# wienkers/marEx

Hardware: AMD Instinct MI355X
Metric: Mcells*timesteps/s, shifting_baseline + hobday_extreme p95 (validation+anomaly+thresholds+mask) (higher is better)
Workload: dtype f32

## Files before the change

### include/marex_hip.h

```cpp
#ifndef MAREX_HIP_H
#define MAREX_HIP_H

#include <stddef.h>
#include <stdint.h>

#ifdef __cplusplus
extern "C" {
#endif

#define MAREX_ABI_VERSION 2
#define MAREX_NDOY 366

typedef struct marex_ctx marex_ctx;

typedef struct marex_thr_stats {
    uint32_t min_key;
    uint32_t max_key;
    uint32_t n_too_low;
    uint32_t n_too_high;
    uint32_t n_unresolved;
    uint32_t reserved[3];
} marex_thr_stats;

enum {
// ... 11 lines not shown
    MAREX_K_TAILS = 11,
    MAREX_K_COUNT = 12
};

int marex_abi_version(void);

typedef struct marex_workspace_cfg {
    int64_t T;
    int64_t T_out;
    int64_t C;
    int max_bucket;
    int list_rows;
} marex_workspace_cfg;
enum {
    MAREX_WS_ANOMALY = 0,
    MAREX_WS_EXTREME = 1,
    MAREX_WS_THRESHOLDS = 2,
    MAREX_WS_LISTS = 3,
    MAREX_WS_AUX = 4,
    MAREX_WS_BINS = 5,
    MAREX_WS_PER_CELL = 6,
    MAREX_WS_TOTAL = 7,
    MAREX_WS_COUNT = 8
};
int marex_workspace_bytes(const marex_workspace_cfg* cfg, size_t* bytes);
int marex_create(int device, marex_ctx** out);
int marex_destroy(marex_ctx* ctx);
const char* marex_last_error(marex_ctx* ctx);
int marex_set_stream(marex_ctx* ctx, void* hip_stream);
int marex_sync(marex_ctx* ctx);

int marex_set_option(marex_ctx* ctx, const char* name, int value);
int marex_clear_option(marex_ctx* ctx, const char* name);
int marex_debug_counters(marex_ctx* ctx, uint64_t* out8, int reset);

int marex_timing_enable(marex_ctx* ctx, int on);
int marex_timing_reset(marex_ctx* ctx);
int marex_timing_get(marex_ctx* ctx, int kernel_id, double* total_ms, int64_t* launches);

int marex_synth_sst_f32(marex_ctx* ctx, const float* mean, const float* amp, const uint8_t* hemi,
                        const uint8_t* land, const float* seas , const float* trend ,
                        uint64_t seed, int64_t cell_base, int64_t T, int64_t C, float* x );

int marex_shifting_baseline_f32(marex_ctx* ctx, const float* x, int64_t T, int64_t C,
                                const int32_t* year_plan, int n_cal_years, int W, int S,
                                int write_clim, const float* edges, int nb, int64_t T_out, float* out,
                                uint16_t* bins, uint8_t* mask, int32_t* invalid_count);

int marex_hobday_thresholds_f32(marex_ctx* ctx, const uint16_t* bins, int64_t T_out, int64_t C, int ny,
                                int nx, const int32_t* doy_start, int max_bucket, const float* first_anom,
                                const float* centres, int nb, double q, int wd, int ws,
                                float lower_bound, float upper_bound, int row0, int row1,
                                float* thr_doy_major, marex_thr_stats* stats);

int marex_mask_ge_doy_f32(marex_ctx* ctx, const float* anom, const float* thr_doy_major,
                          const int32_t* doy_start, const int32_t* doy_rows, int64_t T_out, int64_t C,
                          int64_t c0, int64_t c1, uint8_t* extreme, unsigned long long* n_true);

int marex_mask_ge_doy_bins_f32(marex_ctx* ctx, const float* anom, const uint16_t* bins, const float* edges, int nb,
                               const float* thr_doy_major, const int32_t* doy_start, const int32_t* doy_rows, int64_t T_out,
                               int64_t C, int64_t c0, int64_t c1, uint8_t* extreme, unsigned long long* n_true);

int marex_tail_lists(int max_bucket, int list_rows);
int marex_tail_extract_f32(marex_ctx* ctx, const float* anom, int64_t T_out, int64_t C, const int32_t* doy_start,
                           const int32_t* doy_rows, int max_bucket, const float* edges, int nb, int list_rows, void* lists,
                           uint32_t* aux);

// ... 163 lines not shown
```

### marex_amd/_lib.py

```python

from __future__ import annotations

import ctypes as C
import os
from typing import Optional

from .exceptions import DependencyError, ProcessingError

_HERE = os.path.dirname(os.path.abspath(__file__))
LIB_PATH = os.environ.get("MAREX_LIB_PATH") or os.path.join(_HERE, "csrc", "libmarex_hip.so")

_p = C.c_void_p
_i32 = C.c_int
_i64 = C.c_int64
_u64 = C.c_uint64
_f32 = C.c_float
_f64 = C.c_double

PROTOTYPES = {
    "marex_abi_version": (_i32, []),
    "marex_workspace_bytes": (_i32, [_p, _p]),
    "marex_create": (_i32, [_i32, C.POINTER(_p)]),
    "marex_destroy": (_i32, [_p]),
    "marex_last_error": (C.c_char_p, [_p]),
# ... 163 lines not shown
            raise ProcessingError(f"{what} failed (code {rc})", details=msg.decode() if msg else None)

    def set_stream(self, stream_ptr: int) -> None:
        self.check(self.lib.marex_set_stream(self.handle, _p(stream_ptr)), "marex_set_stream")

    def sync(self) -> None:
        self.check(self.lib.marex_sync(self.handle), "marex_sync")

    def set_option(self, name: str, value: Optional[int]) -> None:
        if value is None:
            self.check(self.lib.marex_clear_option(self.handle, name.encode()), "marex_clear_option")
            self.py_opts.pop(name, None)
        else:
            self.check(self.lib.marex_set_option(self.handle, name.encode(), int(value)), "marex_set_option")
            self.py_opts[name] = int(value)

    def options(self, **opts):
        import contextlib

        @contextlib.contextmanager
        def _cm():
            before = {k: self.py_opts.get(k) for k in opts}
            for k, v in opts.items():
                self.set_option(k, v)
            try:
                yield self
            finally:
                for k, old in before.items():
                    self.set_option(k, old)

        return _cm()

    def debug_counters(self, reset: bool = True):
        buf = (C.c_uint64 * 8)()
        self.check(self.lib.marex_debug_counters(self.handle, buf, int(reset)), "marex_debug_counters")
        return [int(v) for v in buf]

    def timing_enable(self, on: bool = True) -> None:
        self.check(self.lib.marex_timing_enable(self.handle, int(on)), "marex_timing_enable")

    def timing_reset(self) -> None:
        self.check(self.lib.marex_timing_reset(self.handle), "marex_timing_reset")

    def timing_get(self, kernel: str):
        ms, n = _f64(0.0), _i64(0)
        self.check(
            self.lib.marex_timing_get(self.handle, KERNEL_IDS[kernel], C.byref(ms), C.byref(n)), "marex_timing_get"
        )
        return ms.value, n.value
```

### marex_amd/csrc/marex_common.hip.h

```cpp
#pragma once
#include <hip/hip_runtime.h>

#include <cmath>
#include <type_traits>
#include <cstdarg>
#include <cstdio>
#include <cstring>
#include <map>
#include <string>
#include <vector>

#include "marex_hip.h"

#define NDOY MAREX_NDOY

struct TimedLaunch {
    int kid;
    hipEvent_t a, b;
};

struct marex_ctx {
    int device = 0;
    hipStream_t stream = nullptr;
    std::string err;
    bool timing = false;
    std::vector<TimedLaunch> pending;
    double total_ms[MAREX_K_COUNT] = {0};
    int64_t launches[MAREX_K_COUNT] = {0};
    int* shift_info = nullptr;
    int* shift_plan = nullptr;
    size_t shift_plan_years = 0;
    int* shift_lplan = nullptr;
    size_t shift_lplan_years = 0;
    unsigned char* thr_scratch = nullptr;
    size_t thr_scratch_bytes = 0;
    unsigned char* detrend_scratch = nullptr;
    size_t detrend_scratch_bytes = 0;
    unsigned char* morph_scratch = nullptr;
    size_t morph_scratch_bytes = 0;
    int n_cu = 0;
    std::map<std::string, int> opts;
    long long* row_off = nullptr;
    size_t row_off_bytes = 0;
    long long* row_off_mask = nullptr;
    size_t row_off_mask_bytes = 0;
    unsigned long long* dbg_counters = nullptr;
};

#define MAREX_DBG_COUNTERS 8

static inline int ctx_opt(marex_ctx* ctx, const char* name, int dflt) {
    auto it = ctx->opts.find(name);
    return it == ctx->opts.end() ? dflt : it->second;
}

#ifdef MAREX_ABLATION
#define MAREX_ABLATE_OPT(ctx, name) ctx_opt(ctx, name, 0)
#else
#define MAREX_ABLATE_OPT(ctx, name) 0
#endif

static inline unsigned long long* ctx_debug_counters(marex_ctx* ctx) {
    if (!ctx->dbg_counters) {
        if (hipMalloc((void**)&ctx->dbg_counters, MAREX_DBG_COUNTERS * sizeof(unsigned long long)) != hipSuccess) return nullptr;
        (void)hipMemsetAsync(ctx->dbg_counters, 0, MAREX_DBG_COUNTERS * sizeof(unsigned long long), ctx->stream);
    }
    return ctx->dbg_counters;
}

static inline int device_cus(marex_ctx* ctx) {
    if (ctx->n_cu <= 0) {
        int n = 0;
        if (hipDeviceGetAttribute(&n, hipDeviceAttributeMultiprocessorCount, ctx->device) != hipSuccess || n <= 0) n = 256;
        ctx->n_cu = n;
    }
    return ctx->n_cu;
}

static inline int fail(marex_ctx* ctx, int code, const char* fmt, ...) {
    char buf[512];
    va_list ap;
    va_start(ap, fmt);
// ... 131 lines not shown
```

### marex_amd/csrc/marex_tails.hip

```cpp
#include "marex_common.hip.h"
#include "marex_tails.hip.h"

typedef __amdgpu_buffer_rsrc_t tl_rsrc_t;
__device__ __forceinline__ tl_rsrc_t tl_make_rsrc(const void* base) {
    return __builtin_amdgcn_make_buffer_rsrc(const_cast<void*>(base), 0, -1, 0x00020000);
}
__device__ __forceinline__ uint4 tl_load_chunk(tl_rsrc_t r, unsigned voff, unsigned soff) {
    typedef unsigned u4 __attribute__((ext_vector_type(4)));
    const u4 v = __builtin_amdgcn_raw_buffer_load_b128(r, (int)voff, (int)soff, 0);
    return make_uint4(v.x, v.y, v.z, v.w);
}
__device__ __forceinline__ unsigned pk_sub_sat_u16(unsigned a, unsigned b) {
    unsigned r;
    asm("v_pk_sub_u16 %0, %1, %2 clamp" : "=v"(r) : "v"(a), "v"(b));
    return r;
}
__device__ __forceinline__ unsigned pk_add_u16(unsigned a, unsigned b) {
    unsigned r;
    asm("v_pk_add_u16 %0, %1, %2" : "=v"(r) : "v"(a), "v"(b));
    return r;
}
__device__ __forceinline__ unsigned pk_sub_u16(unsigned a, unsigned b) {
    unsigned r;
    asm("v_pk_sub_u16 %0, %1, %2" : "=v"(r) : "v"(a), "v"(b));
// ... 303 lines not shown
        cell = (long)j * nx + gi;
    } else {
        cell_valid = icol < nx && !spare;
        cell = icol < nx ? icol : nx - 1;
    }
    if (!cell_valid) cell = 0;
    const bool is_out = !spare && tr >= P && tr < TR - P && tc >= P && tc < TC - P && j < row1 && icol < nx && (ny > 0 ? j >= row0 : true);
    const int d_begin = (int)blockIdx.y * Dd;
    const int ndays = (NDOY - d_begin) < Dd ? (NDOY - d_begin) : Dd;
    const int pd = wd / 2;
    bool land = true;
    if (is_out) land = !(anom[cell] == anom[cell]);
    if (!__syncthreads_or(is_out && !land)) {
        if (is_out)
            for (int dd = 0; dd < ndays; ++dd) thr[(size_t)(d_begin + dd) * C + cell] = nan_f();
        return;
    }
    if (is_out && land)
        for (int dd = 0; dd < ndays; ++dd) thr[(size_t)(d_begin + dd) * C + cell] = nan_f();

    unsigned* mycol = &lev[ci * TT_LS];
    uint2* mycol2 = reinterpret_cast<uint2*>(mycol);
    typedef __attribute__((address_space(3))) unsigned lds_u32;
    const unsigned col_lds = (unsigned)(size_t)(lds_u32*)mycol;
    const int base_max = nb - TT_BW > 0 ? nb - TT_BW : 0;
    auto clamp_base = [&](int b) { return b < 0 ? 0 : (b > base_max ? base_max : b); };
    int B0 = 0;
    int BW = nb < TT_BW ? nb : TT_BW;
    constexpr int NLP = (TT_BW + 2 + 1) / 2;
    const unsigned voff = (unsigned)cell * 16u;
    const unsigned chunk_row = (unsigned)C * 16u;
    const size_t day_stride = (size_t)NPER * nch * (size_t)C;

    auto load_bucket = [&](int d0) {
        TailBucket<NPERT> b;
        b.d = d0;
        const tl_rsrc_t r = tl_make_rsrc(lists + (size_t)d0 * day_stride);
#pragma unroll
        for (int p = 0; p < NPF; ++p)
            b.c0[p] = (p < NPER) ? tl_load_chunk(r, voff, (unsigned)(nch * p) * chunk_row) : make_uint4(0, 0, 0, 0);
        b.aux = aux[(size_t)d0 * C + cell];
        return b;
    };
    auto bump = [&](int k, int sgn) {
        const int odd = k & 1;
        unsigned addr;
        asm("v_lshl_add_u32 %0, %1, 1, %2" : "=v"(addr) : "v"(k - odd), "v"(col_lds));
        int v;
        const int mul = sgn > 0 ? 65535 : -65535, one = sgn > 0 ? 1 : -1;
        asm("v_mad_i32_i24 %0, %1, %2, %3" : "=v"(v) : "v"(odd), "v"(mul), "v"(one));
        __hip_atomic_fetch_add((lds_u32*)(size_t)addr, (unsigned)v, __ATOMIC_RELAXED, __HIP_MEMORY_SCOPE_WORKGROUP);
    };
    int mytot = 0;
    constexpr bool ctx_asm_bump = true;
    auto bump_chunk = [&](const uint4& ch, int n, int sgn, int nfix) {
#pragma unroll
        for (int u = 0; u < 8; ++u) {
            const bool on = n > u;
            if (u >= nfix && __builtin_amdgcn_ballot_w64(on) == 0) break;
            if (on) {
                int lvl = tl_bin1(ch, u) - B0;
                lvl = lvl > BW + 1 ? BW + 1 : lvl;
                bump(lvl, sgn);
            }
        }
    };
    auto apply_bucket = [&](const TailBucket<NPERT>& b, int sgn) {
        const int cnt = cell_valid ? (int)(b.aux & 0x3FFu) : 0;
        const unsigned lim = ((unsigned)(B0 + 1) << TAIL_POS_BITS) - 1u;
        const unsigned lim_rep = lim | (lim << 16);
        const tl_rsrc_t r = tl_make_rsrc(lists + (size_t)b.d * day_stride);
        int n_in = 0;
        auto one_list = [&](const uint4& ch, int p) {
            const int n = cnt > 0 ? tl_count_above(ch, lim_rep) : 0;
            n_in += n;
            if (ctx_asm_bump) { if (sgn > 0) tl_bump_chunk<1>(ch, n, B0, BW + 1, col_lds); else tl_bump_chunk<-1>(ch, n, B0, BW + 1, col_lds); }
            else bump_chunk(ch, n, sgn, NPERT >= 3 ? 2 : 1);
            bool full = n == 8;
#pragma unroll
            for (int jj = 1; jj < 4; ++jj) {
                if (jj >= nch || __builtin_amdgcn_ballot_w64(full) == 0) break;
                const uint4 cj = tl_load_chunk(r, voff, (unsigned)(nch * p + jj) * chunk_row);
                const int nj = full ? tl_count_above(cj, lim_rep) : 0;
                n_in += nj;
                if (ctx_asm_bump) { if (sgn > 0) tl_bump_chunk<1>(cj, nj, B0, BW + 1, col_lds); else tl_bump_chunk<-1>(cj, nj, B0, BW + 1, col_lds); }
                else bump_chunk(cj, nj, sgn, 0);
                full = nj == 8;
            }
        };
#pragma unroll
        for (int p = 0; p < NPF; ++p)
            if (p < NPER) one_list(b.c0[p], p);
#pragma nounroll
        for (int p = NPF; p < NPER; p += 2) {
            const uint4 e0 = tl_load_chunk(r, voff, (unsigned)(nch * p) * chunk_row);
            const uint4 e1 = p + 1 < NPER ? tl_load_chunk(r, voff, (unsigned)(nch * (p + 1)) * chunk_row) : make_uint4(0, 0, 0, 0);
            one_list(e0, p);
            if (p + 1 < NPER) one_list(e1, p + 1);
        }
        const int below = cnt - n_in;
        if (below > 0) __hip_atomic_fetch_add((lds_u32*)(size_t)col_lds, (unsigned)(sgn > 0 ? below : -below), __ATOMIC_RELAXED,
                                              __HIP_MEMORY_SCOPE_WORKGROUP);
        mytot += sgn > 0 ? cnt : -cnt;
    };
    auto prefix = [&]() -> unsigned {
        unsigned run_rep = 0;
#pragma unroll
        for (int i = 0; i < (NLP + 1) / 2; ++i) {
            uint2 w = mycol2[i];
            w.x = pk_add_u16(w.x + (w.x << 16), run_rep);
            run_rep = __builtin_amdgcn_perm(w.x, w.x, 0x03020302u);
            w.y = pk_add_u16(w.y + (w.y << 16), run_rep);
            run_rep = __builtin_amdgcn_perm(w.y, w.y, 0x03020302u);
            mycol2[i] = w;
        }
        return run_rep & 0xFFFFu;
    };
    auto unprefix = [&]() {
        unsigned prev = 0;
#pragma unroll
        for (int i = 0; i < (NLP + 1) / 2; ++i) {
            const uint2 w = mycol2[i];
            uint2 o;
            o.x = pk_sub_u16(w.x, __builtin_amdgcn_alignbit(w.x, prev, 16));
            o.y = pk_sub_u16(w.y, __builtin_amdgcn_alignbit(w.y, w.x, 16));
            prev = w.y;
            mycol2[i] = o;
        }
    };
    auto wrap = [&](int d) { return ((d % NDOY) + NDOY) % NDOY; };
    auto rebuild = [&](int d) {
        for (int r = 0; r < TT_LS / 2; ++r) mycol2[r] = make_uint2(0u, 0u);
        mytot = 0;
        TailBucket<NPERT> cur = load_bucket(wrap(d - pd));
        for (int o = -pd + 1; o <= pd; ++o) {
            const TailBucket<NPERT> nxt = load_bucket(wrap(d + o));
            apply_bucket(cur, +1);
            cur = nxt;
        }
        apply_bucket(cur, +1);
    };
    auto pooled = [&](int k) {
        const unsigned* base = mycol + (k >> 1);
        const int sh16 = (k & 1) * 16;
        int sum = 0;
#pragma unroll
        for (int dr = -P; dr <= P; ++dr)
#pragma unroll
            for (int dc = -P; dc <= P; ++dc) sum += (int)((base[(dr * TC + dc) * TT_LS] >> sh16) & 0xFFFFu);
        return sum;
    };
    auto pooled_tot = [&]() {
        const unsigned* base = &tot_s[tr * TC + tc];
        int sum = 0;
#pragma unroll
        for (int dr = -P; dr <= P; ++dr)
#pragma unroll
            for (int dc = -P; dc <= P; ++dc) sum += (int)base[dr * TC + dc];
        return sum;
    };
    auto window = [&](int start, int (&Wv)[8]) {
        const unsigned* base = mycol + (start >> 1);
        unsigned a0 = 0, a1 = 0, a2 = 0, a3 = 0;
#pragma unroll
        for (int dr = -P; dr <= P; ++dr)
#pragma unroll
            for (int dc = -P; dc <= P; ++dc) {
                const uint2* p2 = reinterpret_cast<const uint2*>(base + (dr * TC + dc) * TT_LS);
                const uint2 u = p2[0], v = p2[1];
// ... 53 lines not shown
        }
    };
    unsigned kmin = 0xFFFFFFFFu, kmax = 0u, nlow = 0u, nhigh = 0u;
    auto emit_threshold = [&](int d, int iu, int ck, int cb, double qpos) {
        const int il = iu > 0 ? iu - 1 : 0;
        const int cs_iu = ck;
        const int cs_il = iu > 0 ? cb : ck;
        const int diff = cs_iu - cs_il;
        const double frac = diff > 0 ? (qpos - (double)cs_il) / (double)diff : 0.5;
        const float dc = centres[iu] - centres[il];
        const double prod = frac * (double)dc;
        float t32 = (float)((double)centres[il] + prod);
        if (iu == 0) t32 = centres[0];
        const unsigned key = ordered_key(t32);
        kmin = key < kmin ? key : kmin;
        kmax = key > kmax ? key : kmax;
        if (t32 > upper_bound) ++nhigh;
        if (t32 < lower_bound) {
            ++nlow;
            t32 = lower_bound;
        }
        thr[(size_t)d * C + cell] = t32;
    };

    if (t == 0) {
        s_est_min = 0x7fffffff;
        s_est_max = -1;
        s_lo[0] = s_lo[1] = s_hi[0] = s_hi[1] = 0;
        s_iumin[0] = s_iumin[1] = 0x7fffffff;
        s_iumax[0] = s_iumax[1] = -1;
    }
    __syncthreads();
    {
        const TailBucket<NPERT> b = load_bucket(d_begin);
        const int cnt = cell_valid ? (int)(b.aux & 0x3FFu) : 0;
        if (cnt > 0) {
            int rank = (int)ceil((1.0 - q) * (double)cnt / (double)NPER);
            rank = rank < 1 ? 1 : (rank > 8 ? 8 : rank);
            unsigned key = 0;
#pragma unroll
            for (int u = 0; u < 8; ++u)
                if (u == rank - 1) key = tl_key(b.c0[0], u);
            if (key != 0u) {
                const int est = (int)(key >> TAIL_POS_BITS) - 1;
                atomicMin(&s_est_min, est);
                atomicMax(&s_est_max, est);
            }
        }
    }
    __syncthreads();
    {
        const int emin = s_est_min, emax = s_est_max;
        if (emax >= 0) {
            const int span = emax - emin + 1;
            B0 = clamp_base(span <= TT_BW - 2 * TT_MARGIN ? emin - (TT_BW - span) / 2 : emin - TT_MARGIN);
        }
    }
    BW = nb - B0 < TT_BW ? nb - B0 : TT_BW;

    int hint = -1;
    bool need_rebuild = true;
    unsigned long long n_rebuild = 0, n_pass = 0;
    TailBucket<NPERT> pin, pout;
    pin.d = pout.d = 0;
    pin.aux = pout.aux = 0;
#pragma unroll
    for (int p = 0; p < NPF; ++p) pin.c0[p] = pout.c0[p] = make_uint4(0, 0, 0, 0);
#ifdef MAREX_STAMPS
    unsigned long long st_p1 = 0, st_p2 = 0, st_bar = 0;
#define STAMP() __builtin_amdgcn_s_memtime()
#endif
    for (int dd = 0; dd < ndays; ++dd) {
        const int d = d_begin + dd;
        const int dpar = dd & 1;
#ifdef MAREX_STAMPS
        const unsigned long long tA = STAMP();
#endif
        if (need_rebuild) {
            rebuild(d);
            need_rebuild = false;
            ++n_rebuild;
            hint = -1;
        } else {
            unprefix();
            apply_bucket(pin, +1);
            apply_bucket(pout, -1);
        }
        tot_s[ci] = prefix();
        if (dd + 1 < ndays) {
            pin = load_bucket(wrap(d + 1 + pd));
            pout = load_bucket(wrap(d - pd));
        }
#ifdef MAREX_STAMPS
        const unsigned long long tB = STAMP();
        st_p1 += tB - tA;
#endif
        bool resolved = !(is_out && !land);
        int tried_lo = B0, tried_hi = B0;
        bool excursion = false;
        for (int pass = 0;; ++pass) {
            const int par = pass & 1;
#ifdef MAREX_STAMPS
            const unsigned long long tC0 = STAMP();
#endif
            __syncthreads();
#ifdef MAREX_STAMPS
            const unsigned long long tC = STAMP();
            st_bar += tC - tC0;
#endif
            if (t == 0) {
                s_lo[par ^ 1] = 0;
                s_hi[par ^ 1] = 0;
                if (pass == 0) {
                    s_iumin[dpar ^ 1] = 0x7fffffff;
                    s_iumax[dpar ^ 1] = -1;
                }
            }
            int iu_lo = 0x7fffffff, iu_hi = -1;
            if (!resolved) {
                const int tot = pooled_tot();
                if (tot > 0) {
                    const double qpos = q * (double)tot;
                    int ck, cb;
                    int k = find_level(hint, BW + 1, qpos, ck, cb);
// ... 77 lines not shown
                }
            }
        }
    }
    for (int sft = 32; sft > 0; sft >>= 1) {
        const unsigned a = __shfl_down(kmin, sft, 64), b = __shfl_down(kmax, sft, 64);
        kmin = a < kmin ? a : kmin;
        kmax = b > kmax ? b : kmax;
        nlow += __shfl_down(nlow, sft, 64);
        nhigh += __shfl_down(nhigh, sft, 64);
    }
    if ((t & 63) == 0) {
        if (kmin != 0xFFFFFFFFu) atomicMin(&stats->min_key, kmin);
        if (kmax != 0u) atomicMax(&stats->max_key, kmax);
        if (nlow) atomicAdd(&stats->n_too_low, nlow);
        if (nhigh) atomicAdd(&stats->n_too_high, nhigh);
    }
#ifdef MAREX_STAMPS
#ifdef MAREX_STAMPS_WAVE
    const int st_wave = MAREX_STAMPS_WAVE >= 0 ? MAREX_STAMPS_WAVE : (int)((blockIdx.x + blockIdx.y) % (NT / 64));
    if (dbg && t == st_wave * 64) {
#else
    if (dbg && t == 0) {
#endif
        atomicAdd(&dbg[5], st_p1);
        atomicAdd(&dbg[6], st_p2);
        atomicAdd(&dbg[7], st_bar);
    }
#endif
    if (dbg && t == 0) {
        atomicAdd(&dbg[0], n_rebuild);
        atomicAdd(&dbg[2], n_pass);
        atomicAdd(&dbg[3], (unsigned long long)ndays);
    }
}

template <int NSC>
__global__ void __launch_bounds__(64)
k_thr_cells(const uint4* __restrict__ lists, const unsigned* __restrict__ aux, int NPER, int nch, const float* __restrict__ anom,
            long C, long c0, long c1, int nblk, const float* __restrict__ centres, int nb, double q, int wd, float lower_bound,
            float upper_bound, float* __restrict__ thr, marex_thr_stats* __restrict__ stats, unsigned long long* __restrict__ dbg) {
    extern __shared__ uint4 ring[];
    const int lane = (int)threadIdx.x;
    const long cell_raw = c0 + (long)blockIdx.x * 64 + lane;
    const bool valid = cell_raw < c1;
    const long cell = valid ? cell_raw : c1 - 1;
    const int d_begin = (int)blockIdx.y * NDOY / nblk, d_end = ((int)blockIdx.y + 1) * NDOY / nblk;
    const bool land = !(anom[cell] == anom[cell]);
    if (__builtin_amdgcn_ballot_w64(valid && !land) == 0) {
        if (valid)
            for (int d = d_begin; d < d_end; ++d) thr[(size_t)d * C + cell] = nan_f();
        return;
    }
    const int pd = wd / 2, nslot = (wd * NPER + 3) & ~3;
    uint4* mine = ring + lane;
    for (int k = wd * NPER; k < nslot; ++k) mine[k * 64] = make_uint4(0, 0, 0, 0);
    const unsigned voff = (unsigned)cell * 16u, chunk_row = (unsigned)C * 16u;
    const size_t day_stride = (size_t)NPER * nch * (size_t)C;
    auto wrap = [](int d) { return d < 0 ? d + NDOY : (d >= NDOY ? d - NDOY : d); };
    auto cnt_of = [&](int day) { return (int)(aux[(size_t)day * C + cell] & 0x3FFu); };
    auto load_day = [&](int day, int k) {
        const tl_rsrc_t r = tl_make_rsrc(lists + (size_t)day * day_stride);
        for (int p = 0; p < NPER; ++p) mine[((k % wd) * NPER + p) * 64] = tl_load_chunk(r, voff, (unsigned)(nch * p) * chunk_row);
    };
    int tot = 0;
    for (int o = 0; o < wd; ++o) {
// ... 239 lines not shown
        else                                                  \
            hipLaunchKernelGGL((k_thr_tails<PP, TCC, NTT, 3, ##__VA_ARGS__>), grid, dim3(NTT), lds_pad, ctx->stream, MAREX_TT_ARGS); \
    } while (0)
    {
        LaunchTimer lt(ctx, MAREX_K_THRESHOLDS);
        if (TR == 1)
            MAREX_TT_LAUNCH(0, 256, 256);
        else if (half)
            MAREX_TT_LAUNCH(2, 32, 512, 16);
        else if (big && p == 1)
            MAREX_TT_LAUNCH(1, 32, 1024);
        else if (big && p == 2 && tall)
            MAREX_TT_LAUNCH(2, 30, 1024, 34);
        else if (big && p == 2)
            MAREX_TT_LAUNCH(2, 32, 1024);
        else if (big)
            MAREX_TT_LAUNCH(3, 32, 1024);
        else if (p == 1)
            MAREX_TT_LAUNCH(1, 16, 256);
        else if (p == 2)
            MAREX_TT_LAUNCH(2, 16, 256);
        else
            MAREX_TT_LAUNCH(3, 16, 256);
    }
#undef MAREX_TT_LAUNCH
#undef MAREX_TT_ARGS
    HIP_TRY(ctx, hipGetLastError());
    return 0;
}

#ifndef MASK_WAVES
#define MASK_WAVES 5
#endif
template <int NPERT>
__global__ void __launch_bounds__(256, MASK_WAVES)
k_mask_tails(const uint4* __restrict__ lists, const unsigned* __restrict__ aux, int NPER_all, int nch, const float* __restrict__ anom,
             const float* __restrict__ edges, int nb, const float* __restrict__ thr, const int* __restrict__ doy_start,
             const int* __restrict__ doy_rows, const long long* __restrict__ row_off, const long long* __restrict__ row_off_anom,
             long C, long c0, long c1, unsigned char* __restrict__ out, unsigned long long* __restrict__ n_true,
             unsigned long long* __restrict__ dbg) {
    const int nchunk = (int)gridDim.y;
    const int dA = (int)blockIdx.y * NDOY / nchunk, dB = ((int)blockIdx.y + 1) * NDOY / nchunk;
    const long c = (c0 & ~255L) + ((long)blockIdx.x * 256 + threadIdx.x) * 4;
    unsigned cnt_true = 0;
    unsigned long long n_slow = 0;
    if (c >= c0 && c < c1) {
        const float inv_width = (float)(nb - 1) / (edges[nb] - edges[1]);
        for (int d = dA; d < dB; ++d) {
            const int r0 = doy_start[d], nd = doy_start[d + 1] - r0;
            if (nd == 0) continue;
            const float4 th4 = *reinterpret_cast<const float4*>(thr + (size_t)d * C + c);
            const float tv[4] = {th4.x, th4.y, th4.z, th4.w};
            const uint4 ax = *reinterpret_cast<const uint4*>(aux + (size_t)d * C + c);
            const unsigned av[4] = {ax.x, ax.y, ax.z, ax.w};
            unsigned beyond = 0;
            unsigned bits[4][4];
            unsigned lim_ge[4];
            int kt[4];
            bool slow = false, walk[4];
#pragma unroll
            for (int i = 0; i < 4; ++i) {
                bits[i][0] = bits[i][1] = bits[i][2] = bits[i][3] = 0u;
                const bool isnum = tv[i] == tv[i];
                kt[i] = isnum ? digitize_bin(tv[i], edges, nb, inv_width) : nb;
                slow = slow || (isnum && (av[i] & TAIL_AUX_BEYOND) && ((av[i] & TAIL_AUX_MANY) || kt[i] >= nb));
                beyond |= (isnum && (av[i] & TAIL_AUX_BEYOND)) ? 1u : 0u;
                walk[i] = isnum && (av[i] & 0x3FFu) > 0 && kt[i] < nb;
                const unsigned lim = ((unsigned)(kt[i] + 1) << TAIL_POS_BITS) - 1u;
                lim_ge[i] = lim | (lim << 16);
            }
            auto set_prefix = [&](const uint4& q, int n, int i) {
#pragma unroll
                for (int u = 0; u < 8; ++u) {
                    const bool on = n > u;
                    if (u >= 1 && __builtin_amdgcn_ballot_w64(on) == 0) break;
                    if (on) {
                        const int pos = (int)(tl_key(q, u) & (TAIL_MAX_BUCKET - 1));
#pragma unroll
                        for (int wi = 0; wi < 4; ++wi)
                            if ((pos >> 5) == wi) bits[i][wi] |= 1u << (pos & 31);
                    }
                }
            };
            if (__builtin_amdgcn_ballot_w64(!slow) != 0)
            for (int pg = 0; pg < NPER_all; pg += NPERT) {
                const int NPER = (NPER_all - pg) < NPERT ? (NPER_all - pg) : NPERT;
                uint4 ch[NPERT][4];
                const uint4* row0 = lists + (((size_t)d * NPER_all + pg) * nch) * C + c;
#pragma unroll
                for (int p = 0; p < NPERT; ++p)
#pragma unroll
                    for (int i = 0; i < 4; ++i) ch[p][i] = p < NPER ? row0[(size_t)(p * nch) * C + i] : make_uint4(0, 0, 0, 0);
            float cand_val[NPERT][4];
            int cand_pos[NPERT][4];
            unsigned redo = 0;
            {
#pragma unroll
                for (int p = 0; p < NPERT; ++p) {
#pragma unroll
                    for (int i = 0; i < 4; ++i) {
                        cand_pos[p][i] = -1;
                        cand_val[p][i] = 0.f;
                        if (p < NPER && walk[i] && !slow) {
                            const unsigned lgt = lim_ge[i] + (0x10001u << TAIL_POS_BITS);
                            const int n_ge = tl_count_above(ch[p][i], lim_ge[i]);
                            const int n_gt = tl_count_above(ch[p][i], lgt);
                            set_prefix(ch[p][i], n_gt, i);
                            if (n_ge == 8 || n_ge - n_gt > 1) redo |= 1u << (p * 4 + i);
                            if (n_ge - n_gt == 1) {
                                const unsigned w[4] = {ch[p][i].x, ch[p][i].y, ch[p][i].z, ch[p][i].w};
                                unsigned lo = w[0], hi = w[1];
#pragma unroll
                                for (int k = 1; k < 4; ++k)
                                    if ((n_gt >> 1) == k) lo = w[k], hi = k < 3 ? w[k + 1] : 0u;
                                const unsigned key = (n_gt & 1) ? (lo >> 16) : (lo & 0xFFFFu);
                                (void)hi;
                                cand_pos[p][i] = (int)(key & (TAIL_MAX_BUCKET - 1));
                            }
                        }
                    }
                }
#pragma unroll
                for (int p = 0; p < NPERT; ++p)
#pragma unroll
                    for (int i = 0; i < 4; ++i)
                        if (cand_pos[p][i] >= 0)
                            cand_val[p][i] = *reinterpret_cast<const float*>(reinterpret_cast<const char*>(anom) + row_off_anom[r0 + cand_pos[p][i]] + (size_t)(c + i) * 4);
#pragma unroll
                for (int p = 0; p < NPERT; ++p)
#pragma unroll
                    for (int i = 0; i < 4; ++i)
                        if (cand_pos[p][i] >= 0 && cand_val[p][i] >= tv[i]) {
                            const int pos = cand_pos[p][i];
#pragma unroll
                            for (int wi = 0; wi < 4; ++wi)
                                if ((pos >> 5) == wi) bits[i][wi] |= 1u << (pos & 31);
                        }
                if (__builtin_amdgcn_ballot_w64(redo != 0u) != 0) {
#pragma unroll
                    for (int p = 0; p < NPERT; ++p)
#pragma unroll
                        for (int i = 0; i < 4; ++i) {
                            if (__builtin_amdgcn_ballot_w64((redo >> (p * 4 + i)) & 1u) == 0) continue;
                            bool on = (redo >> (p * 4 + i)) & 1u;
                            for (int jj = 0; jj < nch; ++jj) {
                                if (__builtin_amdgcn_ballot_w64(on) == 0) break;
                                const uint4 q = on ? row0[(size_t)(p * nch + jj) * C + i] : make_uint4(0, 0, 0, 0);
#pragma unroll
                                for (int u = 0; u < 8; ++u) {
                                    const unsigned key = tl_key(q, u);
                                    const int bin = (int)(key >> TAIL_POS_BITS) - 1, pos = (int)(key & (TAIL_MAX_BUCKET - 1));
                                    on = on && bin >= kt[i];
                                    if (on) {
                                        bool ext = bin > kt[i];
                                        if (!ext) ext = *reinterpret_cast<const float*>(reinterpret_cast<const char*>(anom) + row_off_anom[r0 + pos] + (size_t)(c + i) * 4) >= tv[i];
                                        if (ext) {
#pragma unroll
                                            for (int wi = 0; wi < 4; ++wi)
                                                if ((pos >> 5) == wi) bits[i][wi] |= 1u << (pos & 31);
                                        }
                                    }
                                }
                            }
                        }
                }
            }
            }
            if (__builtin_amdgcn_ballot_w64(beyond != 0u && !slow) != 0) {
#pragma unroll
                for (int i = 0; i < 4; ++i) {
                    if (!slow && tv[i] == tv[i] && (av[i] & TAIL_AUX_BEYOND)) {
                        const int p1 = (int)((av[i] >> 16) & 0x7Fu), p2 = (int)((av[i] >> 23) & 0x7Fu);
                        const bool two = (av[i] & TAIL_AUX_SECOND) != 0u;
#pragma unroll
                        for (int wi = 0; wi < 4; ++wi) {
                            if ((p1 >> 5) == wi) bits[i][wi] |= 1u << (p1 & 31);
                            if (two && (p2 >> 5) == wi) bits[i][wi] |= 1u << (p2 & 31);
                        }
                    }
                }
            }
            if (slow) {
                ++n_slow;
                for (int r = 0; r < nd; ++r) {
                    const size_t off = (size_t)doy_rows[r0 + r] * C + c;
                    const float4 a = *reinterpret_cast<const float4*>(anom + off);
                    const unsigned m0 = a.x >= tv[0], m1 = a.y >= tv[1], m2 = a.z >= tv[2], m3 = a.w >= tv[3];
                    cnt_true += m0 + m1 + m2 + m3;
                    __builtin_nontemporal_store(m0 | (m1 << 8) | (m2 << 16) | (m3 << 24), reinterpret_cast<unsigned*>(out + off));
                }
            } else {
                unsigned char* obase = out + c;
#pragma unroll
                for (int wi = 0; wi < 4; ++wi) {
                    const unsigned b0 = bits[0][wi], b1 = bits[1][wi], b2 = bits[2][wi], b3 = bits[3][wi];
                    cnt_true += __popc(b0) + __popc(b1) + __popc(b2) + __popc(b3);
                    if (wi * 32 >= nd) break;
#pragma unroll
                    for (int g = 0; g < 4; ++g) {
                        const int rlo = wi * 32 + g * 8;
                        if (rlo >= nd) break;
                        const unsigned q0 = b0 >> (g * 8), q1 = b1 >> (g * 8), q2 = b2 >> (g * 8), q3 = b3 >> (g * 8);
                        const long long* ro = row_off + r0 + rlo;
                        if (rlo + 8 <= nd) {
#pragma unroll
                            for (int rr = 0; rr < 8; ++rr) {
                                const unsigned m = ((q0 >> rr) & 1u) | (((q1 >> rr) & 1u) << 8) | (((q2 >> rr) & 1u) << 16) | (((q3 >> rr) & 1u) << 24);
                                __builtin_nontemporal_store(m, reinterpret_cast<unsigned*>(obase + ro[rr]));
                            }
                        } else {
                            for (int rr = 0; rr < nd - rlo; ++rr) {
                                const unsigned m = ((q0 >> rr) & 1u) | (((q1 >> rr) & 1u) << 8) | (((q2 >> rr) & 1u) << 16) | (((q3 >> rr) & 1u) << 24);
                                __builtin_nontemporal_store(m, reinterpret_cast<unsigned*>(obase + ro[rr]));
                            }
                        }
                    }
                }
            }
        }
    }
    if (n_true) {
        for (int s = 32; s > 0; s >>= 1) cnt_true += __shfl_down(cnt_true, s, 64);
        if ((threadIdx.x & 63) == 0 && cnt_true) atomicAdd(n_true, (unsigned long long)cnt_true);
    }
    if (dbg) {
        for (int s = 32; s > 0; s >>= 1) n_slow += __shfl_down(n_slow, s, 64);
        if ((threadIdx.x & 63) == 0 && n_slow) atomicAdd(&dbg[4], n_slow);
    }
}

extern "C" int marex_mask_ge_doy_tails_f32(marex_ctx* ctx, const void* lists, const uint32_t* aux, int list_rows, int max_bucket,
                                           const float* anom,
                                           const float* edges, int nb, const float* thr_doy_major, const int32_t* doy_start,
                                           const int32_t* doy_rows, int64_t T_out, int64_t C, int64_t c0, int64_t c1,
                                           uint8_t* extreme, unsigned long long* n_true) {
    if (!ctx) return -1;
    if (!lists || !aux || !anom || !edges || !thr_doy_major || !doy_start || !doy_rows || !extreme || T_out <= 0 || C <= 0 || nb < 4)
        return fail(ctx, -1, "marex_mask_ge_doy_tails_f32: null pointer or empty shape");
    if (c0 < 0 || c1 > C || c0 >= c1) return fail(ctx, -1, "marex_mask_ge_doy_tails_f32: need 0 <= c0 < c1 <= C");
    int NPER, nch;
    if (!tails_geometry(max_bucket, list_rows, NPER, nch))
        return fail(ctx, -4, "marex_mask_ge_doy_tails_f32: buckets must hold 1..%d rows, lists 8..32 rows", TAIL_MAX_BUCKET);
    const bool vec = (C % 4 == 0) && (c0 % 4 == 0) && (c1 % 4 == 0) && (((uintptr_t)anom | (uintptr_t)thr_doy_major) % 16 == 0) &&
                     ((uintptr_t)extreme % 4 == 0) && ((uintptr_t)aux % 16 == 0) && nb < 0x7fff;
    if (!vec)
        return marex_mask_ge_doy_f32(ctx, anom, thr_doy_major, doy_start, doy_rows, T_out, C, c0, c1, extreme, n_true);
    HIP_TRY(ctx, hipSetDevice(ctx->device));
    {
        LaunchTimer lt(ctx, MAREX_K_MASK);
        const unsigned ncb = (unsigned)(((c1 - (c0 & ~255L)) / 4 + 255) / 256);
        unsigned chunks = (16384 + ncb - 1) / ncb;
        chunks = chunks < MASK_DOY_CHUNKS ? MASK_DOY_CHUNKS : (chunks > 61 ? 61 : chunks);
        {
            const int forced = ctx_opt(ctx, "MASK_CHUNKS", 0);
            if (forced >= 1 && forced <= 366) chunks = (unsigned)forced;
        }
        unsigned long long* dbg = ctx_debug_counters(ctx);
        const uint4* tl = reinterpret_cast<const uint4*>(lists);
        const size_t need = (size_t)T_out * sizeof(long long);
        if (need > ctx->row_off_mask_bytes) {
            if (ctx->row_off_mask) HIP_TRY(ctx, hipFree(ctx->row_off_mask));
            ctx->row_off_mask = nullptr;
            ctx->row_off_mask_bytes = 0;
            HIP_TRY(ctx, hipMalloc((void**)&ctx->row_off_mask, need));
            ctx->row_off_mask_bytes = need;
        }
        hipLaunchKernelGGL(k_row_offsets, dim3((unsigned)((T_out + 255) / 256)), dim3(256), 0, ctx->stream, doy_rows, (long)T_out, (long)C,
                           ctx->row_off_mask, 1);
        const size_t need4 = (size_t)T_out * sizeof(long long);
        if (need4 > ctx->row_off_bytes) {
            if (ctx->row_off) HIP_TRY(ctx, hipFree(ctx->row_off));
            ctx->row_off = nullptr;
            ctx->row_off_bytes = 0;
            HIP_TRY(ctx, hipMalloc((void**)&ctx->row_off, need4));
            ctx->row_off_bytes = need4;
        }
        hipLaunchKernelGGL(k_row_offsets, dim3((unsigned)((T_out + 255) / 256)), dim3(256), 0, ctx->stream, doy_rows, (long)T_out, (long)C,
                           ctx->row_off, (int)sizeof(float));
#define MAREX_MT_ARGS tl, aux, NPER, nch, anom, edges, nb, thr_doy_major, doy_start, doy_rows, ctx->row_off_mask, ctx->row_off, (long)C, (long)c0, (long)c1, extreme, n_true, dbg
        const int grp = ctx_opt(ctx, "MASK_GROUP", 0);
        if (NPER <= 1 || grp == 1)
            hipLaunchKernelGGL(k_mask_tails<1>, dim3(ncb, chunks), dim3(256), 0, ctx->stream, MAREX_MT_ARGS);
        else if ((NPER != 3 && grp != 3) || grp == 2)
            hipLaunchKernelGGL(k_mask_tails<2>, dim3(ncb, chunks), dim3(256), 0, ctx->stream, MAREX_MT_ARGS);
        else
            hipLaunchKernelGGL(k_mask_tails<3>, dim3(ncb, chunks), dim3(256), 0, ctx->stream, MAREX_MT_ARGS);
#undef MAREX_MT_ARGS
    }
    HIP_TRY(ctx, hipGetLastError());
    return 0;
}
```

Measured before the change: 319,500.

## Skip tail-list loads for dead/dry cells and specialise mask bitset width

The threshold kernel pre-scans each cell's aux counts over the reach window and skips all tail-list bucket loads when a cell has no samples. The mask kernel pre-scans thresholds per 4-cell group and skips thr, aux and list loads when every threshold is NaN, so land and invalid cells cost little. The mask kernel also gains a bitset-width template (3 words when buckets hold at most 96 rows), packs candidate positions into a byte-packed register, and switches list loads to buffer-resource loads. The extra pre-scan passes add memory reads for live cells, and the buffer-offset path adds a 32-bit size guard.

```diff
diff --git a/include/marex_hip.h b/include/marex_hip.h
--- a/include/marex_hip.h
+++ b/include/marex_hip.h
@@ -67,7 +67,7 @@
 
 int marex_set_option(marex_ctx* ctx, const char* name, int value);
 int marex_clear_option(marex_ctx* ctx, const char* name);
-int marex_debug_counters(marex_ctx* ctx, uint64_t* out8, int reset);
+int marex_debug_counters(marex_ctx* ctx, uint64_t* out10, int reset);
 
 int marex_timing_enable(marex_ctx* ctx, int on);
 int marex_timing_reset(marex_ctx* ctx);
diff --git a/marex_amd/_lib.py b/marex_amd/_lib.py
--- a/marex_amd/_lib.py
+++ b/marex_amd/_lib.py
@@ -219,7 +219,7 @@
         return _cm()
 
     def debug_counters(self, reset: bool = True):
-        buf = (C.c_uint64 * 8)()
+        buf = (C.c_uint64 * 10)()
         self.check(self.lib.marex_debug_counters(self.handle, buf, int(reset)), "marex_debug_counters")
         return [int(v) for v in buf]
 
diff --git a/marex_amd/csrc/marex_common.hip.h b/marex_amd/csrc/marex_common.hip.h
--- a/marex_amd/csrc/marex_common.hip.h
+++ b/marex_amd/csrc/marex_common.hip.h
@@ -47,7 +47,9 @@
     unsigned long long* dbg_counters = nullptr;
 };
 
-#define MAREX_DBG_COUNTERS 8
+#define MAREX_DBG_COUNTERS 10
+#define MAREX_DBG_MASK_DRY 8
+#define MAREX_DBG_THR_DEAD 9
 
 static inline int ctx_opt(marex_ctx* ctx, const char* name, int dflt) {
     auto it = ctx->opts.find(name);
diff --git a/marex_amd/csrc/marex_tails.hip b/marex_amd/csrc/marex_tails.hip
--- a/marex_amd/csrc/marex_tails.hip
+++ b/marex_amd/csrc/marex_tails.hip
@@ -359,14 +359,36 @@
     const unsigned chunk_row = (unsigned)C * 16u;
     const size_t day_stride = (size_t)NPER * nch * (size_t)C;
 
-    auto load_bucket = [&](int d0) {
+    auto wrap = [&](int d) { return ((d % NDOY) + NDOY) % NDOY; };
+    bool dead = !cell_valid;
+    if (cell_valid) {
+        const int nreach = ndays + 2 * pd;
+        unsigned any = 0;
+        for (int o = 0; o < nreach; o += 8) {
+            unsigned a8[8];
+#pragma unroll
+            for (int k = 0; k < 8; ++k) a8[k] = aux[(size_t)wrap(d_begin - pd + (o + k < nreach ? o + k : nreach - 1)) * C + cell];
+#pragma unroll
+            for (int k = 0; k < 8; ++k) any |= a8[k];
+        }
+        dead = (any & TAIL_AUX_COUNT) == 0u;
+    }
+    auto load_bucket = [&](TailBucket<NPERT>& b, int d0) {
+        b.d = d0;
+        if (!dead) {
+            const tl_rsrc_t r = tl_make_rsrc(lists + (size_t)d0 * day_stride);
+#pragma unroll
+            for (int p = 0; p < NPF; ++p)
+                b.c0[p] = (p < NPER) ? tl_load_chunk(r, voff, (unsigned)(nch * p) * chunk_row) : make_uint4(0, 0, 0, 0);
+            b.aux = aux[(size_t)d0 * C + cell];
+        }
+    };
+    auto empty_bucket = [&]() {
         TailBucket<NPERT> b;
-        b.d = d0;
-        const tl_rsrc_t r = tl_make_rsrc(lists + (size_t)d0 * day_stride);
-#pragma unroll
-        for (int p = 0; p < NPF; ++p)
-            b.c0[p] = (p < NPER) ? tl_load_chunk(r, voff, (unsigned)(nch * p) * chunk_row) : make_uint4(0, 0, 0, 0);
-        b.aux = aux[(size_t)d0 * C + cell];
+        b.d = 0;
+        b.aux = 0;
+#pragma unroll
+        for (int p = 0; p < NPF; ++p) b.c0[p] = make_uint4(0, 0, 0, 0);
         return b;
     };
     auto bump = [&](int k, int sgn) {
@@ -407,7 +429,8 @@
 #pragma unroll
             for (int jj = 1; jj < 4; ++jj) {
                 if (jj >= nch || __builtin_amdgcn_ballot_w64(full) == 0) break;
-                const uint4 cj = tl_load_chunk(r, voff, (unsigned)(nch * p + jj) * chunk_row);
+                uint4 cj = make_uint4(0, 0, 0, 0);
+                if (full) cj = tl_load_chunk(r, voff, (unsigned)(nch * p + jj) * chunk_row);
                 const int nj = full ? tl_count_above(cj, lim_rep) : 0;
                 n_in += nj;
                 if (ctx_asm_bump) { if (sgn > 0) tl_bump_chunk<1>(cj, nj, B0, BW + 1, col_lds); else tl_bump_chunk<-1>(cj, nj, B0, BW + 1, col_lds); }
@@ -420,8 +443,12 @@
             if (p < NPER) one_list(b.c0[p], p);
 #pragma nounroll
         for (int p = NPF; p < NPER; p += 2) {
-            const uint4 e0 = tl_load_chunk(r, voff, (unsigned)(nch * p) * chunk_row);
-            const uint4 e1 = p + 1 < NPER ? tl_load_chunk(r, voff, (unsigned)(nch * (p + 1)) * chunk_row) : make_uint4(0, 0, 0, 0);
+            uint4 e0, e1;
+            asm volatile("" : "=v"(e0.x), "=v"(e0.y), "=v"(e0.z), "=v"(e0.w), "=v"(e1.x), "=v"(e1.y), "=v"(e1.z), "=v"(e1.w));
+            if (!dead) {
+                e0 = tl_load_chunk(r, voff, (unsigned)(nch * p) * chunk_row);
+                if (p + 1 < NPER) e1 = tl_load_chunk(r, voff, (unsigned)(nch * (p + 1)) * chunk_row);
+            }
             one_list(e0, p);
             if (p + 1 < NPER) one_list(e1, p + 1);
         }
@@ -455,13 +482,13 @@
             mycol2[i] = o;
         }
     };
-    auto wrap = [&](int d) { return ((d % NDOY) + NDOY) % NDOY; };
     auto rebuild = [&](int d) {
         for (int r = 0; r < TT_LS / 2; ++r) mycol2[r] = make_uint2(0u, 0u);
         mytot = 0;
-        TailBucket<NPERT> cur = load_bucket(wrap(d - pd));
+        TailBucket<NPERT> cur = empty_bucket(), nxt = empty_bucket();
+        load_bucket(cur, wrap(d - pd));
         for (int o = -pd + 1; o <= pd; ++o) {
-            const TailBucket<NPERT> nxt = load_bucket(wrap(d + o));
+            load_bucket(nxt, wrap(d + o));
             apply_bucket(cur, +1);
             cur = nxt;
         }
@@ -581,7 +608,8 @@
     }
     __syncthreads();
     {
-        const TailBucket<NPERT> b = load_bucket(d_begin);
+        TailBucket<NPERT> b = empty_bucket();
+        load_bucket(b, d_begin);
         const int cnt = cell_valid ? (int)(b.aux & 0x3FFu) : 0;
         if (cnt > 0) {
             int rank = (int)ceil((1.0 - q) * (double)cnt / (double)NPER);
@@ -610,11 +638,7 @@
     int hint = -1;
     bool need_rebuild = true;
     unsigned long long n_rebuild = 0, n_pass = 0;
-    TailBucket<NPERT> pin, pout;
-    pin.d = pout.d = 0;
-    pin.aux = pout.aux = 0;
-#pragma unroll
-    for (int p = 0; p < NPF; ++p) pin.c0[p] = pout.c0[p] = make_uint4(0, 0, 0, 0);
+    TailBucket<NPERT> pin = empty_bucket(), pout = empty_bucket();
 #ifdef MAREX_STAMPS
     unsigned long long st_p1 = 0, st_p2 = 0, st_bar = 0;
 #define STAMP() __builtin_amdgcn_s_memtime()
@@ -637,8 +661,8 @@
         }
         tot_s[ci] = prefix();
         if (dd + 1 < ndays) {
-            pin = load_bucket(wrap(d + 1 + pd));
-            pout = load_bucket(wrap(d - pd));
+            load_bucket(pin, wrap(d + 1 + pd));
+            load_bucket(pout, wrap(d - pd));
         }
 #ifdef MAREX_STAMPS
         const unsigned long long tB = STAMP();
@@ -782,6 +806,10 @@
         atomicAdd(&dbg[0], n_rebuild);
         atomicAdd(&dbg[2], n_pass);
         atomicAdd(&dbg[3], (unsigned long long)ndays);
+    }
+    if (dbg) {
+        const unsigned long long nd64 = __builtin_popcountll(__builtin_amdgcn_ballot_w64(dead && cell_valid));
+        if ((t & 63) == 0 && nd64) atomicAdd(&dbg[MAREX_DBG_THR_DEAD], nd64);
     }
 }
 
@@ -1087,7 +1115,7 @@
 #ifndef MASK_WAVES
 #define MASK_WAVES 5
 #endif
-template <int NPERT>
+template <int NPERT, int NW>
 __global__ void __launch_bounds__(256, MASK_WAVES)
 k_mask_tails(const uint4* __restrict__ lists, const unsigned* __restrict__ aux, int NPER_all, int nch, const float* __restrict__ anom,
              const float* __restrict__ edges, int nb, const float* __restrict__ thr, const int* __restrict__ doy_start,
@@ -1098,31 +1126,66 @@
     const int dA = (int)blockIdx.y * NDOY / nchunk, dB = ((int)blockIdx.y + 1) * NDOY / nchunk;
     const long c = (c0 & ~255L) + ((long)blockIdx.x * 256 + threadIdx.x) * 4;
     unsigned cnt_true = 0;
-    unsigned long long n_slow = 0;
+    unsigned n_slow = 0;
+    bool dry = false;
     if (c >= c0 && c < c1) {
         const float inv_width = (float)(nb - 1) / (edges[nb] - edges[1]);
+        const unsigned voff = (unsigned)c * 16u;
+        const unsigned chunk_row = (unsigned)C * 16u;
+        const size_t day_stride = (size_t)NPER_all * nch * (size_t)C;
+        unsigned numeric = 0;
+        for (int d8 = dA; d8 < dB && !numeric; d8 += 8) {
+            float4 t8[8];
+#pragma unroll
+            for (int k = 0; k < 8; ++k) {
+                const int dk = d8 + k < dB ? d8 + k : dB - 1;
+                t8[k] = *reinterpret_cast<const float4*>(thr + (size_t)dk * C + c);
+            }
+#pragma unroll
+            for (int k = 0; k < 8; ++k)
+                numeric |= (unsigned)(t8[k].x == t8[k].x) | (unsigned)(t8[k].y == t8[k].y) | (unsigned)(t8[k].z == t8[k].z) | (unsigned)(t8[k].w == t8[k].w);
+        }
+        dry = numeric == 0u;
         for (int d = dA; d < dB; ++d) {
             const int r0 = doy_start[d], nd = doy_start[d + 1] - r0;
             if (nd == 0) continue;
-            const float4 th4 = *reinterpret_cast<const float4*>(thr + (size_t)d * C + c);
+            float4 th4 = make_float4(nan_f(), nan_f(), nan_f(), nan_f());
+            uint4 ax = make_uint4(0u, 0u, 0u, 0u);
+            if (!dry) {
+                th4 = *reinterpret_cast<const float4*>(thr + (size_t)d * C + c);
+                ax = *reinterpret_cast<const uint4*>(aux + (size_t)d * C + c);
+            }
             const float tv[4] = {th4.x, th4.y, th4.z, th4.w};
-            const uint4 ax = *reinterpret_cast<const uint4*>(aux + (size_t)d * C + c);
             const unsigned av[4] = {ax.x, ax.y, ax.z, ax.w};
             unsigned beyond = 0;
-            unsigned bits[4][4];
+            unsigned bits[4][NW];
             unsigned lim_ge[4];
-            int kt[4];
-            bool slow = false, walk[4];
+            bool slow = false;
 #pragma unroll
             for (int i = 0; i < 4; ++i) {
-                bits[i][0] = bits[i][1] = bits[i][2] = bits[i][3] = 0u;
+#pragma unroll
+                for (int wi = 0; wi < NW; ++wi) bits[i][wi] = 0u;
                 const bool isnum = tv[i] == tv[i];
-                kt[i] = isnum ? digitize_bin(tv[i], edges, nb, inv_width) : nb;
-                slow = slow || (isnum && (av[i] & TAIL_AUX_BEYOND) && ((av[i] & TAIL_AUX_MANY) || kt[i] >= nb));
+                const int kt = isnum ? digitize_bin(tv[i], edges, nb, inv_width) : nb;
+                slow = slow || (isnum && (av[i] & TAIL_AUX_BEYOND) && ((av[i] & TAIL_AUX_MANY) || kt >= nb));
                 beyond |= (isnum && (av[i] & TAIL_AUX_BEYOND)) ? 1u : 0u;
-                walk[i] = isnum && (av[i] & 0x3FFu) > 0 && kt[i] < nb;
-                const unsigned lim = ((unsigned)(kt[i] + 1) << TAIL_POS_BITS) - 1u;
+                const bool walk = isnum && (av[i] & 0x3FFu) > 0 && kt < nb;
+                const unsigned lim = walk ? ((unsigned)(kt + 1) << TAIL_POS_BITS) - 1u : 0xFFFFu;
                 lim_ge[i] = lim | (lim << 16);
+            }
+            if (__builtin_amdgcn_ballot_w64(beyond != 0u && !slow) != 0) {
+#pragma unroll
+                for (int i = 0; i < 4; ++i) {
+                    if (!slow && tv[i] == tv[i] && (av[i] & TAIL_AUX_BEYOND)) {
+                        const int p1 = (int)((av[i] >> 16) & 0x7Fu), p2 = (int)((av[i] >> 23) & 0x7Fu);
+                        const bool two = (av[i] & TAIL_AUX_SECOND) != 0u;
+#pragma unroll
+                        for (int wi = 0; wi < NW; ++wi) {
+                            if ((p1 >> 5) == wi) bits[i][wi] |= 1u << (p1 & 31);
+                            if (two && (p2 >> 5) == wi) bits[i][wi] |= 1u << (p2 & 31);
+                        }
+                    }
+                }
             }
             auto set_prefix = [&](const uint4& q, int n, int i) {
 #pragma unroll
@@ -1132,31 +1195,31 @@
                     if (on) {
                         const int pos = (int)(tl_key(q, u) & (TAIL_MAX_BUCKET - 1));
 #pragma unroll
-                        for (int wi = 0; wi < 4; ++wi)
+                        for (int wi = 0; wi < NW; ++wi)
                             if ((pos >> 5) == wi) bits[i][wi] |= 1u << (pos & 31);
                     }
                 }
             };
-            if (__builtin_amdgcn_ballot_w64(!slow) != 0)
+            const tl_rsrc_t rl = tl_make_rsrc(lists + (size_t)d * day_stride);
+            if (__builtin_amdgcn_ballot_w64(!slow && !dry) != 0)
             for (int pg = 0; pg < NPER_all; pg += NPERT) {
                 const int NPER = (NPER_all - pg) < NPERT ? (NPER_all - pg) : NPERT;
                 uint4 ch[NPERT][4];
-                const uint4* row0 = lists + (((size_t)d * NPER_all + pg) * nch) * C + c;
 #pragma unroll
                 for (int p = 0; p < NPERT; ++p)
 #pragma unroll
-                    for (int i = 0; i < 4; ++i) ch[p][i] = p < NPER ? row0[(size_t)(p * nch) * C + i] : make_uint4(0, 0, 0, 0);
+                    for (int i = 0; i < 4; ++i)
+                        ch[p][i] = (p < NPER && !dry) ? tl_load_chunk(rl, voff + 16u * i, (unsigned)((pg + p) * nch) * chunk_row) : make_uint4(0, 0, 0, 0);
             float cand_val[NPERT][4];
-            int cand_pos[NPERT][4];
+            unsigned cand_pos[NPERT];
             unsigned redo = 0;
             {
 #pragma unroll
                 for (int p = 0; p < NPERT; ++p) {
+                    cand_pos[p] = 0xFFFFFFFFu;
 #pragma unroll
                     for (int i = 0; i < 4; ++i) {
-                        cand_pos[p][i] = -1;
-                        cand_val[p][i] = 0.f;
-                        if (p < NPER && walk[i] && !slow) {
+                        if (p < NPER && lim_ge[i] != 0xFFFFFFFFu && !slow) {
                             const unsigned lgt = lim_ge[i] + (0x10001u << TAIL_POS_BITS);
                             const int n_ge = tl_count_above(ch[p][i], lim_ge[i]);
                             const int n_gt = tl_count_above(ch[p][i], lgt);
@@ -1170,7 +1233,7 @@
                                     if ((n_gt >> 1) == k) lo = w[k], hi = k < 3 ? w[k + 1] : 0u;
                                 const unsigned key = (n_gt & 1) ? (lo >> 16) : (lo & 0xFFFFu);
                                 (void)hi;
-                                cand_pos[p][i] = (int)(key & (TAIL_MAX_BUCKET - 1));
+                                cand_pos[p] ^= ((key & (TAIL_MAX_BUCKET - 1)) ^ 0xFFu) << (8 * i);
                             }
                         }
                     }
@@ -1178,19 +1241,23 @@
 #pragma unroll
                 for (int p = 0; p < NPERT; ++p)
 #pragma unroll
-                    for (int i = 0; i < 4; ++i)
-                        if (cand_pos[p][i] >= 0)
-                            cand_val[p][i] = *reinterpret_cast<const float*>(reinterpret_cast<const char*>(anom) + row_off_anom[r0 + cand_pos[p][i]] + (size_t)(c + i) * 4);
+                    for (int i = 0; i < 4; ++i) {
+                        const unsigned pos = __builtin_amdgcn_ubfe(cand_pos[p], 8 * i, 8);
+                        cand_val[p][i] = 0.f;
+                        if (pos != 0xFFu)
+                            cand_val[p][i] = *reinterpret_cast<const float*>(reinterpret_cast<const char*>(anom) + row_off_anom[r0 + (int)pos] + (size_t)(c + i) * 4);
+                    }
 #pragma unroll
                 for (int p = 0; p < NPERT; ++p)
 #pragma unroll
-                    for (int i = 0; i < 4; ++i)
-                        if (cand_pos[p][i] >= 0 && cand_val[p][i] >= tv[i]) {
-                            const int pos = cand_pos[p][i];
-#pragma unroll
-                            for (int wi = 0; wi < 4; ++wi)
+                    for (int i = 0; i < 4; ++i) {
+                        const int pos = (int)__builtin_amdgcn_ubfe(cand_pos[p], 8 * i, 8);
+                        if (pos != 0xFF && cand_val[p][i] >= tv[i]) {
+#pragma unroll
+                            for (int wi = 0; wi < NW; ++wi)
                                 if ((pos >> 5) == wi) bits[i][wi] |= 1u << (pos & 31);
                         }
+                    }
                 if (__builtin_amdgcn_ballot_w64(redo != 0u) != 0) {
 #pragma unroll
                     for (int p = 0; p < NPERT; ++p)
@@ -1198,20 +1265,21 @@
                         for (int i = 0; i < 4; ++i) {
                             if (__builtin_amdgcn_ballot_w64((redo >> (p * 4 + i)) & 1u) == 0) continue;
                             bool on = (redo >> (p * 4 + i)) & 1u;
+                            const int kt = (int)(((lim_ge[i] & 0xFFFFu) + 1u) >> TAIL_POS_BITS) - 1;
                             for (int jj = 0; jj < nch; ++jj) {
                                 if (__builtin_amdgcn_ballot_w64(on) == 0) break;
-                                const uint4 q = on ? row0[(size_t)(p * nch + jj) * C + i] : make_uint4(0, 0, 0, 0);
+                                const uint4 q = on ? tl_load_chunk(rl, voff + 16u * i, (unsigned)((pg + p) * nch + jj) * chunk_row) : make_uint4(0, 0, 0, 0);
 #pragma unroll
                                 for (int u = 0; u < 8; ++u) {
                                     const unsigned key = tl_key(q, u);
                                     const int bin = (int)(key >> TAIL_POS_BITS) - 1, pos = (int)(key & (TAIL_MAX_BUCKET - 1));
-                                    on = on && bin >= kt[i];
+                                    on = on && bin >= kt;
                                     if (on) {
-                                        bool ext = bin > kt[i];
+                                        bool ext = bin > kt;
                                         if (!ext) ext = *reinterpret_cast<const float*>(reinterpret_cast<const char*>(anom) + row_off_anom[r0 + pos] + (size_t)(c + i) * 4) >= tv[i];
                                         if (ext) {
 #pragma unroll
-                                            for (int wi = 0; wi < 4; ++wi)
+                                            for (int wi = 0; wi < NW; ++wi)
                                                 if ((pos >> 5) == wi) bits[i][wi] |= 1u << (pos & 31);
                                         }
                                     }
@@ -1220,20 +1288,6 @@
                         }
                 }
             }
-            }
-            if (__builtin_amdgcn_ballot_w64(beyond != 0u && !slow) != 0) {
-#pragma unroll
-                for (int i = 0; i < 4; ++i) {
-                    if (!slow && tv[i] == tv[i] && (av[i] & TAIL_AUX_BEYOND)) {
-                        const int p1 = (int)((av[i] >> 16) & 0x7Fu), p2 = (int)((av[i] >> 23) & 0x7Fu);
-                        const bool two = (av[i] & TAIL_AUX_SECOND) != 0u;
-#pragma unroll
-                        for (int wi = 0; wi < 4; ++wi) {
-                            if ((p1 >> 5) == wi) bits[i][wi] |= 1u << (p1 & 31);
-                            if (two && (p2 >> 5) == wi) bits[i][wi] |= 1u << (p2 & 31);
-                        }
-                    }
-                }
             }
             if (slow) {
                 ++n_slow;
@@ -1247,7 +1301,7 @@
             } else {
                 unsigned char* obase = out + c;
 #pragma unroll
-                for (int wi = 0; wi < 4; ++wi) {
+                for (int wi = 0; wi < NW; ++wi) {
                     const unsigned b0 = bits[0][wi], b1 = bits[1][wi], b2 = bits[2][wi], b3 = bits[3][wi];
                     cnt_true += __popc(b0) + __popc(b1) + __popc(b2) + __popc(b3);
                     if (wi * 32 >= nd) break;
@@ -1280,7 +1334,9 @@
     }
     if (dbg) {
         for (int s = 32; s > 0; s >>= 1) n_slow += __shfl_down(n_slow, s, 64);
-        if ((threadIdx.x & 63) == 0 && n_slow) atomicAdd(&dbg[4], n_slow);
+        if ((threadIdx.x & 63) == 0 && n_slow) atomicAdd(&dbg[4], (unsigned long long)n_slow);
+        const unsigned long long n_dry = __builtin_popcountll(__builtin_amdgcn_ballot_w64(dry));
+        if ((threadIdx.x & 63) == 0 && n_dry) atomicAdd(&dbg[MAREX_DBG_MASK_DRY], n_dry);
     }
 }
 
@@ -1297,7 +1353,8 @@
     if (!tails_geometry(max_bucket, list_rows, NPER, nch))
         return fail(ctx, -4, "marex_mask_ge_doy_tails_f32: buckets must hold 1..%d rows, lists 8..32 rows", TAIL_MAX_BUCKET);
     const bool vec = (C % 4 == 0) && (c0 % 4 == 0) && (c1 % 4 == 0) && (((uintptr_t)anom | (uintptr_t)thr_doy_major) % 16 == 0) &&
-                     ((uintptr_t)extreme % 4 == 0) && ((uintptr_t)aux % 16 == 0) && nb < 0x7fff;
+                     ((uintptr_t)extreme % 4 == 0) && ((uintptr_t)aux % 16 == 0) && nb < 0x7fff &&
+                     (int64_t)C * 16 * nch * NPER < (1ll << 32);
     if (!vec)
         return marex_mask_ge_doy_f32(ctx, anom, thr_doy_major, doy_start, doy_rows, T_out, C, c0, c1, extreme, n_true);
     HIP_TRY(ctx, hipSetDevice(ctx->device));
@@ -1334,12 +1391,21 @@
                            ctx->row_off, (int)sizeof(float));
 #define MAREX_MT_ARGS tl, aux, NPER, nch, anom, edges, nb, thr_doy_major, doy_start, doy_rows, ctx->row_off_mask, ctx->row_off, (long)C, (long)c0, (long)c1, extreme, n_true, dbg
         const int grp = ctx_opt(ctx, "MASK_GROUP", 0);
+        const bool w3 = max_bucket <= 96;
+#define MAREX_MT_LAUNCH(G)                                                                                                \
+    do {                                                                                                                  \
+        if (w3)                                                                                                           \
+            hipLaunchKernelGGL((k_mask_tails<G, 3>), dim3(ncb, chunks), dim3(256), 0, ctx->stream, MAREX_MT_ARGS);         \
+        else                                                                                                              \
+            hipLaunchKernelGGL((k_mask_tails<G, 4>), dim3(ncb, chunks), dim3(256), 0, ctx->stream, MAREX_MT_ARGS);         \
+    } while (0)
         if (NPER <= 1 || grp == 1)
-            hipLaunchKernelGGL(k_mask_tails<1>, dim3(ncb, chunks), dim3(256), 0, ctx->stream, MAREX_MT_ARGS);
+            MAREX_MT_LAUNCH(1);
         else if ((NPER != 3 && grp != 3) || grp == 2)
-            hipLaunchKernelGGL(k_mask_tails<2>, dim3(ncb, chunks), dim3(256), 0, ctx->stream, MAREX_MT_ARGS);
+            MAREX_MT_LAUNCH(2);
         else
-            hipLaunchKernelGGL(k_mask_tails<3>, dim3(ncb, chunks), dim3(256), 0, ctx->stream, MAREX_MT_ARGS);
+            MAREX_MT_LAUNCH(3);
+#undef MAREX_MT_LAUNCH
 #undef MAREX_MT_ARGS
     }
     HIP_TRY(ctx, hipGetLastError());
```

Measured after the change: 322,200, median of 6. About the same (+0.8%).
